# ishine/zerovox.cpp

Hardware: AMD Instinct MI355X
Metric: audio-seconds/wall-second (xRT) end-to-end phoneme->22.05 kHz wav (higher is better)
Workload: dtype f16*f16->f32 (MFMA) convs, f32 (MFMA) attention/linear, f32 activations

## Files before the change

### zerovox.cpp_amd/csrc/capi.cpp

```cpp
#include <algorithm>
#include <cmath>
#include <cstring>
#include <map>
#include <optional>
#include <string>
#include <thread>
#include <vector>

#include "common.h"
#include "model.h"
#include "knobs.h"

using zv::Model;

struct PendingBatch;
struct zv_model
{
    Model        *m;
    PendingBatch *pending;
};

static void free_pending(zv_model *m);
static void lane0_select(zv_model *m);
static void use_lane0(zv_model *m);
// ... 968 lines not shown
    if (env)
    {
        bt.d_env_gain = (const float *)(d_in + i_eg);
        bt.d_env = (const int32_t *)(d_in + i_env);
        bt.d_nframes = (const int32_t *)(io + o_nf);
    }
    int32_t *d_nf = (int32_t *)(io + o_nf), *d_ids = (int32_t *)(d_in + i_ids), *d_pun = (int32_t *)(d_in + i_pun);
    float *d_sty = (float *)(d_in + i_sty), *d_hid = (float *)(io + o_hid), *d_mel = (float *)(io + o_mel), *d_wav = (float *)(io + o_wav);
    int32_t *h_nf = (int32_t *)(pin + p_nf), *h_cum = dur ? (int32_t *)(pin + p_cum) : nullptr;
    char *h_wav = pin + p_wav;
    zv_level *h_lvl = vol ? (zv_level *)(pin + p_lvl) : nullptr;
    zv_frame_level *h_cfr = ctr_f ? (zv_frame_level *)(pin + p_cfr) : nullptr, *h_cph = ctr_p ? (zv_frame_level *)(pin + p_cph) : nullptr;
    zv_pitch_frame *h_pfr = pit_f ? (zv_pitch_frame *)(pin + p_pfr) : nullptr;
    zv_pitch_phoneme *h_pph = pit_p ? (zv_pitch_phoneme *)(pin + p_pph) : nullptr;
    float *h_bfr = bnd_f ? (float *)(pin + p_bfr) : nullptr, *h_bph = bnd_p ? (float *)(pin + p_bph) : nullptr;
    const size_t brs = zv::BANDS_ROW_STRIDE;
    auto contour_download = [&](uint32_t u0, uint32_t u1, hipStream_t st) {
        const size_t f0 = pb.woff[u0] / (hop * 4), f1 = u1 < r.count ? pb.woff[u1] / (hop * 4) : frame_rows;
        const size_t n0 = pb.noff[u0], n1 = pb.noff[u1];
        if (h_cfr && f1 > f0)
            ZV_HIP(hipMemcpyAsync(h_cfr + f0, bt.d_ctr_frames + f0, (f1 - f0) * sizeof(zv_frame_level), hipMemcpyDeviceToHost, st));
        if (h_cph && n1 > n0)
            ZV_HIP(hipMemcpyAsync(h_cph + n0, bt.d_ctr_phonemes + n0, (n1 - n0) * sizeof(zv_frame_level), hipMemcpyDeviceToHost, st));
        if (h_pfr && f1 > f0)
            ZV_HIP(hipMemcpyAsync(h_pfr + f0, bt.d_pit_frames + f0, (f1 - f0) * sizeof(zv_pitch_frame), hipMemcpyDeviceToHost, st));
        if (h_pph && n1 > n0)
            ZV_HIP(hipMemcpyAsync(h_pph + n0, bt.d_pit_phonemes + n0, (n1 - n0) * sizeof(zv_pitch_phoneme), hipMemcpyDeviceToHost, st));
        if (h_bfr && f1 > f0)
            ZV_HIP(hipMemcpyAsync(h_bfr + f0 * brs, bt.d_bnd_frames + f0 * brs, (f1 - f0) * brs * 4, hipMemcpyDeviceToHost, st));
        if (h_bph && n1 > n0)
            ZV_HIP(hipMemcpyAsync(h_bph + n0 * brs, bt.d_bnd_phonemes + n0 * brs, (n1 - n0) * brs * 4, hipMemcpyDeviceToHost, st));
    };
    const int G = zv::voc_tail_groups(bt.nseg, wav_bytes, M.profiling, M.dbg_layer.kind >= 0);
    try
    {
        hipStream_t cs = M.copy_stream();
        pb.gb.assign(G + 1, r.count);
        pb.gb[0] = 0;
        const uint64_t seq = M.next_batch_seq();
        ZV_HIP(hipEventRecord(M.batch_event(seq, 0), M.stream()));
        if (G <= 1)
        {
            M.chain_dev(bt, d_ids, d_pun, d_sty, d_hid, d_mel, d_wav, d_nf, h_in, d_in, b_in);
            ZV_HIP(hipEventRecord(M.batch_event(seq, 1), M.stream()));
            ZV_HIP(hipMemcpyAsync(h_nf, d_nf, (size_t)bt.nseg * 4, hipMemcpyDeviceToHost, M.stream()));
            if (dur) ZV_HIP(hipMemcpyAsync(h_cum, bt.d_cum, (size_t)ntot * 4, hipMemcpyDeviceToHost, M.stream()));
            ZV_HIP(hipMemcpyAsync(h_wav, d_wav, wav_bytes, hipMemcpyDeviceToHost, M.stream()));
            if (vol) ZV_HIP(hipMemcpyAsync(h_lvl, io + o_lvl, (size_t)bt.nseg * sizeof(zv_level), hipMemcpyDeviceToHost, M.stream()));
            contour_download(0, r.count, M.stream());
            ZV_HIP(hipEventRecord(M.tail_event(1), M.stream()));
        }
        else
        {
            M.chain_dev(bt, d_ids, d_pun, d_sty, d_hid, d_mel, d_wav, d_nf, h_in, d_in, b_in, 1);
            ZV_HIP(hipMemcpyAsync(h_nf, d_nf, (size_t)bt.nseg * 4, hipMemcpyDeviceToHost, M.stream()));
            if (dur) ZV_HIP(hipMemcpyAsync(h_cum, bt.d_cum, (size_t)ntot * 4, hipMemcpyDeviceToHost, M.stream()));
            for (int g = 1; g < G; g++)
            {
                uint32_t u = pb.gb[g - 1] + 1;
                while (u < r.count && pb.woff[u] < wav_bytes * g / G) u++;
                pb.gb[g] = std::min(u, r.count - (uint32_t)(G - g));
            }
            for (int g = 0; g < G; g++)
            {
                const uint32_t u0 = pb.gb[g], u1 = pb.gb[g + 1];
                M.vocode_tail(bt, d_mel, d_wav, (int)u0, (int)(u1 - u0));
                const size_t o0 = pb.woff[u0], o1 = u1 < r.count ? pb.woff[u1] : wav_bytes;
                ZV_HIP(hipEventRecord(M.tail_event(2 * g), M.stream()));
                ZV_HIP(hipStreamWaitEvent(cs, M.tail_event(2 * g), 0));
                ZV_HIP(hipMemcpyAsync(h_wav + o0, (const char *)d_wav + o0, o1 - o0, hipMemcpyDeviceToHost, cs));
                contour_download(u0, u1, cs);
                ZV_HIP(hipEventRecord(M.tail_event(2 * g + 1), cs));
            }
            ZV_HIP(hipEventRecord(M.batch_event(seq, 1), M.stream()));
            if (vol) ZV_HIP(hipMemcpyAsync(h_lvl, io + o_lvl, (size_t)bt.nseg * sizeof(zv_level), hipMemcpyDeviceToHost, M.stream()));
        }
    }
    catch (...)
    {
        hipStreamSynchronize(M.stream());
        if (M.copy_stream()) hipStreamSynchronize(M.copy_stream());
        throw;
    }
    pb.active = true;
    pb.n_utt = r.count;
    pb.G = G;
    pb.T.assign(r.T, r.T + r.count);
    pb.wav.assign(r.out, r.out + r.count);
    pb.n_frames = r.n_frames;
    pb.h_wav = h_wav;
    pb.h_nf = h_nf;
    pb.hop = hop;
    pb.h_cum = h_cum;
    pb.h_lvl = h_lvl;
    pb.levels = r.levels;
    pb.h_cfr = h_cfr;
    pb.h_cph = h_cph;
    if (ctr) pb.contour.assign(r.contour, r.contour + r.count);
    else pb.contour.clear();
    pb.h_pfr = h_pfr;
    pb.h_pph = h_pph;
    if (pit) pb.pitch.assign(r.pitch, r.pitch + r.count);
    else pb.pitch.clear();
    pb.h_bfr = h_bfr;
    pb.h_bph = h_bph;
    if (bnd) pb.bands.assign(r.bands, r.bands + r.count);
    else pb.bands.clear();
    pb.N.assign(r.n, r.n + r.count);
    if (dur) pb.dur.assign(r.durations, r.durations + r.count);
    else pb.dur.clear();
}

static void batch_finish(zv_model *m, int lane)
{
    Model &M = *m->m;
    PendingBatch &pb = pending_slot(m, lane);
    if (!pb.active) zv::fail(ZV_ERR_ARG, "lane %d has no batch in flight", lane);
    M.select_lane(lane);
    try
    {
        for (int g = 0; g < pb.G; g++)
        {
            ZV_HIP(hipEventSynchronize(M.tail_event(2 * g + 1)));
            scatter_out(pb.h_wav, pb.woff.data(), pb.wav.data(), pb.T.data(), pb.hop, pb.gb[g], pb.gb[g + 1]);
        }
        M.sync();
    }
    catch (...)
// ... 879 lines not shown
```

### zerovox.cpp_amd/csrc/knobs.h

```cpp
#pragma once

namespace zv
{

#define ZV_KNOB_LIST(X)                                                                                                               \
    X(ZV_NO_FUSE, 0)                                                                  \
    X(ZV_NO_TRIPLE, 0)                                                                          \
    X(ZV_FUSE256, 0)                                                \
    X(ZV_NO_MERGE, 0)                                                               \
    X(ZV_MERGE_ALWAYS, 0)                 \
    X(ZV_MERGE_SEQ, 1)          \
    X(ZV_MERGE_MAXC, 256)                                  \
    X(ZV_TAIL_GROUPS, 8)                                                        \
    X(ZV_ARENA_FILL, 0)                                         \
    X(ZV_DEC_PREPASS, -1)                                      \
    X(ZV_CONV_MT, 0)                                                              \
    X(ZV_CONV_NT, 0)                                                     \
    X(ZV_CONV_SINGLE, 1)                                    \
    X(ZV_CONV_GEMM, 1)                  \
    X(ZV_CONV_STREAM, 1)        \
    X(ZV_VOC_RUNS, 1)           \
    X(ZV_DEC_RUNS, 1)           \
    X(ZV_DEC_PACK, 1)           \
    X(ZV_UP_GEMM, 1)           \
    X(ZV_GEMM_ORDER, 2)         \
    X(ZV_PAIR_MT, 0)                                                                  \
    X(ZV_CONV_XCD, 1)           \
    X(ZV_CONV_WARM, 1)          \
    X(ZV_LINEAR_MERGED, 1)      \
    X(ZV_BLOCK64, 3)            \
    X(ZV_PAIR64_RING, 1)               \
    X(ZV_TRIPLE_V2, 1)                               \
    X(ZV_TRIPLE_DB, 1)                                                                     \
    X(ZV_TRIPLE_INTERLEAVE, 1)                                                               \
    X(ZV_ATT_SCALAR, 0)                                                                               \
    X(ZV_ATT_MFMA, 0)                                                          \
    X(ZV_LN_TAIL, 1)

#ifdef ZV_DIAG
#define ZV_KNOB_LIST_DIAG(X)                                                                                                          \
    X(ZV_DBG, 0)                                                                       \
    X(ZV_LDS_PAD, 0)            \
    X(ZV_STAMP_CP, 0)                               \
    X(ZV_STAMP_CONV, 0)                                    \
    X(ZV_STAMP_CIN, 0)
#else
#define ZV_KNOB_LIST_DIAG(X)
#endif

enum Knob : int
{
#define ZV_KNOB_ENUM(n, d) n,
    ZV_KNOB_LIST(ZV_KNOB_ENUM)
    ZV_KNOB_LIST_DIAG(ZV_KNOB_ENUM)
#undef ZV_KNOB_ENUM
    ZV_KNOB_COUNT
};

int         knob(Knob k);
bool        knob_set(const char *name, int value);
void        knob_reset();
bool        knob_get(const char *name, int *value);
unsigned    knob_epoch();
const char *knob_name(int k);
#ifdef ZV_DIAG
inline int diag_bits() { return knob(ZV_DBG); }
#else
// ... 5 lines not shown
```

### zerovox.cpp_amd/csrc/model.cpp

```cpp
#include "schedule.h"

#include <algorithm>

namespace zv
{

Model::~Model()
{
    hipSetDevice(device);
    for (Lane &l : lanes_) hipStreamSynchronize(l.stream);
    drop_graphs();
    prof_clear();
    for (void *p : allocs_) hipFree(p);
    for (hipEvent_t e : batch_events_)
        if (e) hipEventDestroy(e);
    for (Lane &l : lanes_)
    {
        if (l.copy_stream) hipStreamSynchronize(l.copy_stream);
        if (l.arena.base) hipFree(l.arena.base);
        if (l.io) hipFree(l.io);
        if (l.pinned) hipHostFree(l.pinned);
        for (hipEvent_t e : l.tail_events) hipEventDestroy(e);
        if (l.copy_stream) hipStreamDestroy(l.copy_stream);
        if (l.stream) hipStreamDestroy(l.stream);
// ... 233 lines not shown
    for (auto &g : graphs_)
        if (g.exec) hipGraphExecDestroy(g.exec);
    graphs_.clear();
}

template <typename F> void Model::run_captured(int kind, const Batch &b, const void *const (&key)[CapturedGraph::NKEY], F &&enqueue)
{
    for (auto &g : graphs_)
        if (g.kind == kind && g.epoch == knob_epoch() && b.same_schedule(g.b) && memcmp(g.p, key, sizeof(key)) == 0)
        {
            ZV_HIP(hipGraphLaunch(g.exec, stream()));
            lane().runs_tab = g.runs_tab;
            lane().runs_n = g.runs_n;
            return;
        }
    reserve_batch(b);
    hipGraph_t graph = nullptr;
    lane().runs_tab = nullptr;
    lane().runs_n = 0;
    ZV_HIP(hipStreamBeginCapture(stream(), hipStreamCaptureModeThreadLocal));
    try
    {
        enqueue();
    }
    catch (...)
    {
        hipStreamEndCapture(stream(), &graph);
        if (graph) hipGraphDestroy(graph);
        throw;
    }
    ZV_HIP(hipStreamEndCapture(stream(), &graph));
    CapturedGraph cg;
    cg.kind = kind;
    cg.epoch = knob_epoch();
    cg.b = b;
    memcpy(cg.p, key, sizeof(key));
    cg.runs_tab = lane().runs_tab;
    cg.runs_n = lane().runs_n;
    hipError_t e = hipGraphInstantiate(&cg.exec, graph, nullptr, nullptr, 0);
    hipGraphDestroy(graph);
    if (e != hipSuccess) fail(ZV_ERR_DEVICE, "hipGraphInstantiate failed: %s", hipGetErrorString(e));
    if (graphs_.size() >= 16)
    {
        ZV_HIP(hipStreamSynchronize(stream()));
        drop_graphs();
    }
    graphs_.push_back(cg);
    ZV_HIP(hipGraphLaunch(cg.exec, stream()));
}

void Model::chain_dev(const Batch &b, const int32_t *d_ids, const int32_t *d_puncts, const float *d_styles, float *d_hidden,
                      float *d_mel, float *d_wav, int32_t *d_nframes, const void *h2d_src, void *h2d_dst, size_t h2d_bytes, int voc_part)
{
    auto run = [&]() {
        if (h2d_bytes) ZV_HIP(hipMemcpyAsync(h2d_dst, h2d_src, h2d_bytes, hipMemcpyHostToDevice, stream()));
        encode_dev(b, d_ids, d_puncts, d_styles, d_hidden, d_nframes);
        decode_dev(b, d_hidden, d_styles, d_mel);
        if (voc_part == 1) vocode_group(b, d_mel, d_wav, 1);
        else vocode_dev(b, d_mel, d_wav);
    };
    if (!graph_mode || profiling) return run();
    const void *key[CapturedGraph::NKEY] = {d_ids, d_puncts, d_styles, d_hidden, d_mel, d_wav, d_nframes, h2d_src};
    run_captured(voc_part == 1 ? 2 : 1, b, key, run);
}

void Model::vocode_dev_graph(const Batch &b, const float *d_mel, float *d_wav)
{
    if (!graph_mode || profiling) return vocode_dev(b, d_mel, d_wav);
    const void *key[CapturedGraph::NKEY] = {d_mel, d_wav};
    run_captured(0, b, key, [&]() { vocode_dev(b, d_mel, d_wav); });
}

}
```

### zerovox.cpp_amd/csrc/model.h

```cpp
#pragma once

#include <cstdint>
#include <cstring>
#include <string>
#include <vector>

#include "common.h"
#include "gguf_reader.h"
#include "kernels.h"

namespace zv
{

struct ConvW
{
    void  *w = nullptr;
    void  *w8 = nullptr;
    float *bias = nullptr;
    int    K = 0, Cin = 0, Cout = 0, Cin_p = 0, Cout_p = 0, ck = 0;
};

struct DeviceArena
{
    char  *base = nullptr;
// ... 49 lines not shown
    const void         *d_bnd_table = nullptr;
    const uint32_t     *d_flt_par = nullptr;

    static Batch single(uint32_t N, uint32_t T, uint32_t num_phonemes)
    {
        Batch b;
        b.n_max = (int)N;
        b.n_real = (int)N;
        b.t_max = (int)T;
        b.n_rows = N;
        b.t_rows = T;
        b.tok1 = Seg{0, (int32_t)N, (int32_t)num_phonemes, 0};
        b.frm1 = Seg{0, (int32_t)T, 0, 0};
        return b;
    }
    Segs tokens() const { return Segs{d_tok, nseg, n_max, tok1}; }
    Segs tokens_merged() const { return d_tok ? Segs{d_tok + nseg, 1, (int)n_rows, tok1} : tokens(); }
    Segs frames_cap() const { return Segs{d_frm, nseg, t_max, frm1}; }
    Segs frames() const { return d_frm_live ? Segs{d_frm_live, nseg, t_max, frm1} : frames_cap(); }
    bool same_schedule(const Batch &o) const
    {
        return nseg == o.nseg && n_max == o.n_max && t_max == o.t_max && n_rows == o.n_rows && t_rows == o.t_rows && d_tok == o.d_tok &&
               d_frm == o.d_frm && (d_tok || memcmp(&tok1, &o.tok1, sizeof(Seg)) == 0) && (d_frm || memcmp(&frm1, &o.frm1, sizeof(Seg)) == 0) &&
               d_ctl == o.d_ctl && d_pctl == o.d_pctl && d_cum == o.d_cum && d_frm_live == o.d_frm_live && has_targets == o.has_targets &&
               d_dec_runs == o.d_dec_runs && d_vol == o.d_vol && d_levels == o.d_levels && d_nframes == o.d_nframes && d_env_gain == o.d_env_gain &&
               d_env == o.d_env && d_ctr_frames == o.d_ctr_frames && d_ctr_phonemes == o.d_ctr_phonemes &&
               d_pit_frames == o.d_pit_frames && d_pit_phonemes == o.d_pit_phonemes && d_pit_par == o.d_pit_par &&
               d_bnd_frames == o.d_bnd_frames && d_bnd_phonemes == o.d_bnd_phonemes && d_bnd_slab == o.d_bnd_slab && d_bnd_par == o.d_bnd_par &&
               d_bnd_table == o.d_bnd_table && d_flt_par == o.d_flt_par;
    }
};

struct CapturedGraph
{
    static constexpr int NKEY = 8;
    int            kind = 0;
    unsigned       epoch = 0;
    Batch          b;
    const void    *p[NKEY] = {};
    hipGraphExec_t exec = nullptr;
    const Seg     *runs_tab = nullptr;
    int            runs_n = 0;
};

class Model
{
  public:
    Model(const std::string &gguf_path, int device);
    ~Model();

    zv_hparams hp{};
    int        device = 0;
    int        n_cu = 256;
    hipStream_t stream() const { return lanes_[cur_lane_].stream; }

    void vocode_dev(const Batch &b, const float *d_mel, float *d_wav);
    void vocode_group(const Batch &b, const float *d_mel, float *d_wav, int part = 0, int seg0 = 0);
    void vocode_tail(const Batch &b, const float *d_mel, float *d_wav, int g0, int cnt);
    hipStream_t copy_stream();
    hipEvent_t  tail_event(int i);
    static constexpr int BATCH_RING = 64;
    uint64_t    next_batch_seq() { return batch_seq_++; }
    uint64_t    batch_seq() const { return batch_seq_; }
    hipEvent_t  batch_event(uint64_t seq, int which);
    void decode_dev(const Batch &b, const float *d_hidden, const float *d_styles, float *d_mel);
    struct EncoderTaps
    {
        float   *features = nullptr, *logdur = nullptr, *pitch = nullptr, *energy = nullptr;
        int32_t *pitch_bucket = nullptr, *energy_bucket = nullptr, *cum = nullptr;
    };
    EncoderTaps encode_dev(const Batch &b, const int32_t *d_ids, const int32_t *d_puncts, const float *d_styles,
                           float *d_hidden, int32_t *d_nframes);

    struct DebugLayer
    {
        int          kind = -1, index = 0;
        const float *x = nullptr;
        float       *out = nullptr;
        bool         done = false;
    } dbg_layer;

    uint32_t max_phonemes() const { return (uint32_t)enc_.posenc_rows; }
    void reserve(uint32_t max_phonemes, uint32_t max_frames);
    void reserve_batch(const Batch &b);
    int  voc_stage_rate(int stage) const;
    int  voc_stage_channels(int stage) const;
    uint32_t max_frames_per_utterance() const;
    int wemb_rows() const { return enc_.wemb_rows; }
    int pemb_rows() const { return enc_.pemb_rows; }
    uint32_t vocoder_halo_frames() const;
    bool voc_runs_off = false;
    bool voc_runs_on(const Batch &b) const;
    const Seg *voc_runs_last(int *n) { *n = lane().runs_n; return lane().runs_tab; }
    DecPlan dec_plan(const Batch &b) const
    {
        return zv::dec_plan(b.nseg, b.t_max, b.t_rows, b.d_frm_live != nullptr, dbg_layer.kind >= 0, b.d_dec_runs != nullptr);
    }
    int  dec_reach_frames() const;
    void sync();

    void select_lane(int i);
    int  selected_lane() const { return cur_lane_; }
    void sync_all_lanes();
    void poison_lane(int i, int byte, size_t filled[3]);

    const void *bands_table();

    void *io_scratch(size_t bytes);
    void *pinned_scratch(size_t bytes);

    bool graph_mode = false;
// ... 90 lines not shown
    };
    size_t level_slab_entries(const Batch &b) const;
    size_t env_knot_entries(const Batch &b) const;
    struct DecLayout
    {
        int    nblk, hs, ss;
        int    rows, nblk_all;
        float *h, *st_x, *st_t, *st_y, *st_a, *cat, *t1, *sc, *x0, *xa, *asr_t;
        double *part_t, *part_o; _Float16 *xa16, *t16, *xr16;
        float *mel_c;
    };
    struct EncLayout { int Vp; float *x, *y, *qkv, *o, *f, *va, *vb; _Float16 *hh; EncoderTaps t; };
    VocLayout voc_layout(DeviceArena &a, const Batch &b) const;
    DecLayout dec_layout(DeviceArena &a, const Batch &b) const;
    EncLayout enc_layout(DeviceArena &a, const Batch &b) const;
    static constexpr size_t ARENA_TAIL = (size_t)1 << 20;
    size_t arena_bytes_for(const Batch &b) const;
    void  arena_require(size_t bytes);
    DeviceArena &stage_arena(const Batch &b);

    void conv(const ConvJob *jobs, int n, const Segs &segs, int rate, const char *name, double bytes, double flops);
    void dbg_inject(void *dev, int ld, int cols, size_t rows);
    void dbg_extract(const void *dev, int ld, int cols, size_t rows);
    ConvJob job(const ConvW &w) const;
    void tick(hipEvent_t *e0);
    void tock(hipEvent_t e0, const char *name, double bytes, double flops);
    void group_begin();
    void group_end(const char *name);
    bool       in_group_ = false;
    hipEvent_t group_e0_ = nullptr;
    double     group_bytes_ = 0.0, group_flops_ = 0.0;
    int        group_n_ = 0;

    struct Lane
    {
        hipStream_t stream = nullptr;
        DeviceArena arena;
        void       *io = nullptr;
        size_t      io_cap = 0;
        void       *pinned = nullptr;
        size_t      pinned_cap = 0;
        hipStream_t copy_stream = nullptr;
        std::vector<hipEvent_t> tail_events;
        const Seg  *runs_tab = nullptr;
        int         runs_n = 0;
    };
    std::vector<Lane> lanes_;
    int  cur_lane_ = 0;
    Lane &lane() { return lanes_[cur_lane_]; }
    uint64_t   batch_seq_ = 0;
    hipEvent_t batch_events_[2 * BATCH_RING] = {};

    bool skip_launch_ = false;
    std::vector<CapturedGraph> graphs_;
    void drop_graphs();
    template <typename F> void run_captured(int kind, const Batch &b, const void *const (&key)[CapturedGraph::NKEY], F &&enqueue);
};

}
```

### zerovox.cpp_amd/csrc/voc_plan.h

```cpp
#pragma once

#include <stddef.h>

#include "conv_plan.h"
#include "knobs.h"

namespace zv
{

constexpr int VOC_MAX_STAGES = 8, VOC_MAX_DIL = 8, VOC_BRANCHES = 3;
struct VocPairGeom
{
    int  k1, k2;
    bool fused, ring, x16;
};
struct VocStageGeom
{
    int         scale;
    int         Cp;
    bool        up_gemm;
    int         up_Cin_p;
    VocPairGeom pair[VOC_BRANCHES][VOC_MAX_DIL];
};
struct VocGeom
// ... 53 lines not shown
    const long Lbatch = (long)c.t_max * rate * c.nseg;
    p.up_pass = !(i == 0 && c0_f16) && voc_up_gemm(s, L) && (size_t)s.up_Cin_p * 2 * L <= Lo * Cp * 4;

    p.all_fusable = true;
    for (int jb = 0; jb < VOC_BRANCHES; jb++)
        for (int d = 0; d < g.n_dil; d++) p.all_fusable = p.all_fusable && s.pair[jb][d].fused;
    p.enough_rows = Cp != 256 || knob(ZV_FUSE256) != 0 || (Lbatch / 54) * 3 >= (long)c.n_cu;
    p.fused = knob(ZV_NO_FUSE) == 0 && p.all_fusable && p.enough_rows;

    p.whole_block = p.fused && knob(ZV_NO_TRIPLE) == 0 && g.n_dil <= TRIPLE_MAX_DIL;
    for (int jb = 0; jb < VOC_BRANCHES && p.whole_block; jb++)
    {
        const int K = s.pair[jb][0].k1;
        p.whole_block = triple_supported(Cp, K, g.dil, g.n_dil);
        for (int d = 0; d < g.n_dil && p.whole_block; d++) p.whole_block = s.pair[jb][d].fused && s.pair[jb][d].k1 == K && s.pair[jb][d].k2 == K;
    }

    const int k64 = knob(ZV_BLOCK64), kmax64 = k64 < 0 ? -k64 : k64;
    if (p.fused && !p.whole_block && Cp == 64 && g.n_dil == 3 && kmax64 >= 3 && (k64 < 0 || Lbatch / 244 >= 4L * c.n_cu))
        for (int jb = 0; jb < VOC_BRANCHES; jb++)
        {
            const VocPairGeom *rp = s.pair[jb];
            const bool one_k = rp[1].k1 == rp[0].k1 && rp[0].k2 == rp[0].k1 && rp[1].k2 == rp[0].k1;
            p.block64[jb] = one_k && rp[0].k1 <= kmax64 && rp[0].ring && rp[1].ring && block64_supported(Cp, rp[0].k1, g.dil, 2);
        }

    const int  merge_tile = Cp >= 256 ? 54 : (Cp == 128 ? 118 : 246);
    const bool merge_pays = knob(ZV_MERGE_ALWAYS) != 0 || (Lbatch / merge_tile >= 4L * c.n_cu && Cp <= knob(ZV_MERGE_MAXC));
    const bool merge = p.fused && !p.whole_block && knob(ZV_NO_MERGE) == 0 && c.dbg_stage != i && merge_pays;
    p.merge = !merge ? VOC_MERGE_NONE : (Cp >= 256 && knob(ZV_MERGE_SEQ) != 0 ? VOC_MERGE_SEQ : VOC_MERGE_ONE);
    return p;
}

inline VocPlan voc_plan(const VocGeom &g, const VocCall &c)
{
    VocPlan p{};
    p.runs = voc_runs(c);
    p.c0_f16 = !c.dbg_active && g.n_up > 0 && voc_up_gemm(g.st[0], c.t_rows) && g.st[0].up_Cin_p == g.in_Cout_p;
    for (int i = 0; i < g.n_up; i++) p.st[i] = voc_plan_stage(g, i, c, p.c0_f16);
    return p;
}

constexpr size_t TAIL_GROUPS_MIN_BYTES = (size_t)16 << 20;
inline int voc_tail_groups(int sw, int nseg, size_t wav_bytes, bool profiling, bool dbg_active)
{
    if (sw <= 1 || nseg < 4 || wav_bytes < TAIL_GROUPS_MIN_BYTES || profiling || dbg_active) return 1;
    return sw < nseg / 2 ? sw : nseg / 2;
}
inline int voc_tail_groups(int nseg, size_t wav_bytes, bool profiling, bool dbg_active)
{
    return voc_tail_groups(knob(ZV_TAIL_GROUPS), nseg, wav_bytes, profiling, dbg_active);
}

}
```

### zerovox.cpp_amd/csrc/vocoder.cpp

```cpp
#include "schedule.h"

#include <algorithm>
#include <cmath>

namespace zv
{

uint32_t Model::vocoder_halo_frames() const
{
    double frames = (voc_.in_conv.K - 1) / 2;
    double rate = 1.0;
    for (int i = 0; i < voc_.n_up; i++)
    {
        frames += (double)voc_.ups[i].K / rate;
        rate *= voc_.scales[i];
        int reach = 0;
        for (int j = 0; j < voc_.n_rb; j++)
        {
            int r = 0;
            for (int d = 0; d < voc_.n_dil; d++)
            {
                const ResPair &rp = voc_.pairs[((size_t)i * voc_.n_rb + j) * voc_.n_dil + d];
                r += (rp.c1.K - 1) / 2 * voc_.dil[d] + (rp.c2.K - 1) / 2;
            }
// ... 18 lines not shown
{
    VocLayout v{};
    v.c0 = a.take_n<float>(bt.t_rows * voc_.in_conv.Cout_p);
    DeviceArena pool[2] = {DeviceArena::counter(), DeviceArena::counter()};
    for (int pass = 0; pass < 2; pass++)
    {
        size_t L = bt.t_rows, need[2] = {0, 0};
        for (int i = 0; i < voc_.n_up; i++)
        {
            DeviceArena &p = pool[i & 1];
            VocLayout::Stage &s = v.st[i];
            L *= voc_.scales[i];
            const size_t n = L * round_up(voc_.in_conv.Cout >> (i + 1), 16);
            p.used = 0;
            s.ub = p.take_n<float>(n);
            for (int j = 0; j < 3; j++) s.y[j] = p.take_n<float>(n);
            for (int j = 0; j < 3; j++) s.xt[j] = (_Float16 *)p.take_n<float>(n);
            need[i & 1] = std::max(need[i & 1], p.used);
        }
        for (int k = 0; k < 2 && pass == 0; k++) pool[k] = DeviceArena{(char *)a.take(need[k]), need[k], 0};
    }
    v.mel_c = a.take_n<float>(bt.t_rows * hp.audio_num_mels);
    v.eq = a.take_n<int32_t>(bt.t_rows);
    v.level_slab = a.take(level_slab_entries(bt) * 16);
    v.env_knots = a.take_n<uint32_t>(env_knot_entries(bt));
    v.contour_slab = a.take(bt.t_rows * 16);
    v.pitch_slab = a.take(bt.t_rows * sizeof(PitchSlabRow));
    v.filter_in = bt.d_flt_par ? a.take_n<float>(bt.t_rows * hp.audio_hop_size) : nullptr;
    v.runs = a.take_n<Seg>(bt.nseg);
    return v;
}

size_t Model::level_slab_entries(const Batch &bt) const
{
    return (bt.t_rows * hp.audio_hop_size + LEVEL_CHUNK_SAMPLES - 1) / LEVEL_CHUNK_SAMPLES + bt.t_rows / (size_t)std::max(bt.t_max, 1) + 1;
}

size_t Model::env_knot_entries(const Batch &bt) const { return bt.t_rows + bt.t_rows / (size_t)std::max(bt.t_max, 1) + 1; }

void Model::vocode_dev(const Batch &bt, const float *d_mel, float *d_wav)
{
    if (bt.t_rows == 0 || bt.t_max <= 0) fail(ZV_ERR_ARG, "T must be > 0");
    vocode_group(bt, d_mel, d_wav);
}

VocCall Model::voc_call(const Batch &bt) const
{
    return VocCall{bt.nseg, bt.t_max, bt.t_rows, n_cu, bt.d_frm_live != nullptr, voc_runs_off, dbg_layer.kind >= 0,
                   dbg_layer.kind == 0 ? dbg_layer.index / voc_.n_rb : -1};
}

bool Model::voc_runs_on(const Batch &bt) const { return voc_runs(voc_call(bt)); }

void Model::vocode_tail(const Batch &bt, const float *d_mel, float *d_wav, int g0, int cnt)
{
    if (!bt.d_frm || g0 < 0 || cnt < 1 || g0 + cnt > bt.nseg) fail(ZV_ERR_ARG, "internal: bad segment group");
    Batch sub = bt;
    sub.d_frm = bt.d_frm + g0;
    if (bt.d_frm_live) sub.d_frm_live = bt.d_frm_live + g0;
    if (bt.d_vol)
    {
        sub.d_vol = bt.d_vol + (size_t)g0 * LEVEL_VOL_STRIDE;
        sub.d_levels = bt.d_levels + g0;
    }
    if (bt.d_nframes) sub.d_nframes = bt.d_nframes + g0;
    if (bt.d_pit_par) sub.d_pit_par = bt.d_pit_par + (size_t)g0 * PITCH_PARAM_STRIDE;
    if (bt.d_bnd_par) sub.d_bnd_par = bt.d_bnd_par + (size_t)g0 * BANDS_PARAM_STRIDE;
    if (bt.d_flt_par) sub.d_flt_par = bt.d_flt_par + (size_t)g0 * FILTER_PARAM_STRIDE;
    if (bt.d_env) sub.d_env = bt.d_env + (size_t)g0 * ENV_CTL_STRIDE;
    sub.nseg = cnt;
    vocode_group(sub, d_mel, d_wav, 2, g0);
}

TripleJob Model::block_job(const ResPair *rp, int n_dil, bool ring, const float *y, float *out) const
{
    TripleJob t;
    memset(&t, 0, sizeof(t));
    t.y = y;
    t.out = out;
    t.n_dil = n_dil;
    t.Cp = rp[0].c1.Cout_p;
    t.K = rp[0].c1.K;
    t.slope = 0.1f;
    for (int d = 0; d < n_dil; d++)
    {
        t.w1[d] = ring ? rp[d].r1 : rp[d].p1;
        t.w2[d] = ring ? rp[d].r2 : rp[d].p2;
        if (!ring)
        {
            t.w1x[d] = rp[d].x1;
            t.w2x[d] = rp[d].x2;
        }
        t.b1[d] = rp[d].c1.bias;
        t.b2[d] = rp[d].c2.bias;
        t.dil[d] = voc_.dil[d];
    }
    return t;
}

Model::DilPairJobs Model::pair_jobs(const ResPair &rp, int dil, const float *yin, float *yout, _Float16 *xt, float *y) const
{
    DilPairJobs r;
    r.c1 = job(rp.c1);
    r.c1.x0 = yin;
    r.c1.pro = PRO_ACT;
    r.c1.slope = 0.1f;
    r.c1.dil = dil;
    r.c1.pad = (rp.c1.K - 1) / 2 * dil;
    r.c1.eact = 1;
    r.c1.oslope = 0.1f;
    r.c1.out_f16 = 1;
    r.c1.out = xt;
    r.c2 = job(rp.c2);
    r.c2.x0 = xt;
    r.c2.pro = PRO_RAW_F16;
    r.c2.res = yin;
    r.c2.ldres = rp.c1.Cout_p;
    r.c2.out = y;
    memset(&r.p, 0, sizeof(r.p));
    r.p.y = yin;
    r.p.out = yout;
    r.p.w1 = rp.x1;
    r.p.w2 = rp.x2;
    r.p.w1r = rp.r1;
    r.p.w2r = rp.r2;
    r.p.b1 = rp.c1.bias;
    r.p.b2 = rp.c2.bias;
    r.p.Cp = rp.c1.Cout_p;
    r.p.K = rp.c1.K;
    r.p.dil = dil;
    r.p.slope = 0.1f;
    return r;
}

void Model::vocode_group(const Batch &bt, const float *d_mel, float *d_wav, int part, int seg0)
{
    struct Unskip { bool &f; ~Unskip() { f = false; } } unskip{skip_launch_};
    skip_launch_ = part == 2;
    const VocLayout lay = voc_layout(stage_arena(bt), bt);
    const int M = hp.audio_num_mels;
    const VocPlan plan = voc_plan(voc_geom_, voc_call(bt));
    const bool runs = plan.runs;
    const Segs fr = runs ? Segs{lay.runs + seg0, bt.nseg, bt.t_max, bt.frm1} : bt.frames();
    if (part != 2)
    {
        lane().runs_tab = runs ? lay.runs : nullptr;
        lane().runs_n = runs ? bt.nseg : 0;
    }
    if (runs)
    {
        ZV_LAUNCH("voc_runs", 12.0 * bt.t_rows * M, 0.0,
                  launch_voc_runs(stream(), d_mel, M, lay.mel_c, lay.eq, lay.runs, bt.frames_cap(), (int)vocoder_halo_frames()));
        d_mel = lay.mel_c;
    }
    size_t L = bt.t_rows;
    double La = std::min((double)bt.t_rows, (double)bt.t_max * bt.nseg);
    if (runs && profiling)
    {
        std::vector<Seg> tab((size_t)bt.nseg);
        ZV_HIP(hipMemcpyAsync(tab.data(), lay.runs + seg0, tab.size() * sizeof(Seg), hipMemcpyDeviceToHost, stream()));
        ZV_HIP(hipStreamSynchronize(stream()));
        La = 0;
        for (const Seg &g : tab) La += g.rows;
    }
    int rate = 1;
    int C = voc_.in_conv.Cout;
    float *c0 = lay.c0;

    {
        ConvJob j = job(voc_.in_conv);
        j.x0 = d_mel;
        j.ldx = M;
        j.pro = PRO_MELNORM;
        j.pa = voc_.mean;
        j.pb = voc_.scale;
        j.out = c0;
        if (plan.c0_f16)
        {
            j.eact = 1;
            j.oslope = 0.1f;
            j.out_f16 = 1;
        }
        conv(&j, 1, fr, rate, "voc_input_conv", conv_bytes(La, M, C, j.K, false), conv_flops(La, M, C, j.K));
        if (dbg_layer.kind == ZV_LAYER_VOC_INPUT)
        {
            dbg_extract(c0, voc_.in_conv.Cout_p, C, L);
            return;
        }
    }

    const float third = (float)(1.0 / (float)voc_.n_rb);
    const float *prev_y[3] = {nullptr, nullptr, nullptr};
    const float *prev_merged = nullptr;
    for (int i = 0; i < voc_.n_up; i++)
    {
        const bool last_stage = i == voc_.n_up - 1;
        const VocStagePlan &sp = plan.st[i];
        skip_launch_ = part == 2;
        const int s = voc_.scales[i];
        const ConvW &up = voc_.ups[i];
        const int Cout = C >> 1, Cp = round_up(Cout, 16);
        const size_t Lo = L * s;
        float *ub = lay.st[i].ub;
        float *y[3] = {lay.st[i].y[0], lay.st[i].y[1], lay.st[i].y[2]};
        _Float16 *const *xt = lay.st[i].xt;

        {
            ConvJob j = job(up);
            j.slope = 0.1f;
            if (i == 0) { j.x0 = c0; j.pro = PRO_ACT; }
            else if (prev_merged) { j.x0 = prev_merged; j.pro = PRO_SCALE_ACT; j.pscale = third; }
            else { j.x0 = prev_y[0]; j.x1 = prev_y[1]; j.x2 = prev_y[2]; j.pro = PRO_SUM3_ACT; j.pscale = third; }
            const bool dbg_up = dbg_layer.kind == ZV_LAYER_VOC_UPSAMPLE && dbg_layer.index == i;
            if (dbg_up)
            {
                float *in = i == 0 ? c0 : const_cast<float *>(prev_merged ? prev_merged : prev_y[0]);
                dbg_inject(in, up.Cin_p, C, L);
                j.x0 = in;
                j.x1 = j.x2 = nullptr;
                if (i > 0) { j.pro = PRO_SCALE_ACT; j.pscale = 1.0f; }
            }
            j.out = ub;
            if (i == 0 && plan.c0_f16)
            {
                j.x0 = c0;
                j.pro = PRO_RAW_F16;
            }
            else if (sp.up_pass)
            {
                ZV_LAUNCH("voc_upsample", 0.0, 0.0, launch_act_f16(stream(), (const float *)j.x0, (const float *)j.x1, (const float *)j.x2,
                                                                   j.pro == PRO_ACT ? 1.0f : j.pscale, j.slope, xt[2], (size_t)L * up.Cin_p));
                j.x0 = xt[2];
                j.x1 = j.x2 = nullptr;
                j.pro = PRO_RAW_F16;
                j.pscale = 1.0f;
            }
            conv(&j, 1, fr, rate, "voc_upsample", 4.0 * La * C * (i == 0 ? 1 : 3) + 4.0 * La * s * Cout + 2.0 * C * Cout * 2 * s,
                 2.0 * La * C * Cout * 2 * s);
        }
        if (dbg_layer.kind == ZV_LAYER_VOC_UPSAMPLE && dbg_layer.index == i)
        {
            dbg_extract(ub, Cp, Cout, Lo);
            return;
        }
        skip_launch_ = (part == 1 && last_stage) || (part == 2 && !last_stage);
        L = Lo;
        La *= s;
        rate *= s;
        C = Cout;
        const bool dbg_here = dbg_layer.kind == 0 && dbg_layer.index / voc_.n_rb == i;
        if (dbg_here) dbg_inject(ub, Cp, Cout, L);
        const ResPair *const rps = &voc_.pairs[(size_t)i * voc_.n_rb * voc_.n_dil];
        const float *ycur[3] = {ub, ub, ub};
        const float *merged_sum = nullptr;
        auto block_cost = [&](const ResPair *rp, int n, double &bytes, double &flops) {
            for (int d = 0; d < n; d++)
            {
                bytes += conv_bytes(La, C, C, rp[d].c1.K, false) + conv_bytes(La, C, C, rp[d].c2.K, true);
                flops += conv_flops(La, C, C, rp[d].c1.K) + conv_flops(La, C, C, rp[d].c2.K);
            }
        };
        group_begin();
        if (sp.whole_block)
        {
            TripleJob tj[3];
            double bb = 0, ff = 0;
            for (int jb = 0; jb < 3; jb++)
            {
                tj[jb] = block_job(rps + jb * voc_.n_dil, voc_.n_dil, false, ub, y[jb]);
                block_cost(rps + jb * voc_.n_dil, voc_.n_dil, bb, ff);
                ycur[jb] = y[jb];
            }
            ZV_LAUNCH("voc_resblock_conv", bb, ff, launch_triple(stream(), tj, 3, n_cu, fr, rate));
        }
        {
            TripleJob tj[3];
            int nj = 0;
            double bb = 0, ff = 0;
            for (int jb = 0; jb < 3; jb++)
            {
                if (!sp.block64[jb]) continue;
                tj[nj++] = block_job(rps + jb * voc_.n_dil, 2, true, ub, (float *)xt[jb]);
                block_cost(rps + jb * voc_.n_dil, 2, bb, ff);
                ycur[jb] = (float *)xt[jb];
            }
            if (nj) ZV_LAUNCH("voc_resblock_conv", bb, ff, launch_block64(stream(), tj, nj, fr, rate));
        }
        for (int d = 0; d < voc_.n_dil && !sp.whole_block; d++)
        {
            ConvJob j1[3], j2[3];
            PairJob pj[3];
            double b1 = 0, f1 = 0, b2 = 0, f2 = 0;
            int npj = 0;
            for (int jb = 0; jb < 3; jb++)
            {
                if (sp.block64[jb] && d < 2) continue;
                const ResPair &rp = rps[jb * voc_.n_dil + d];
                float *yout = sp.fused ? ((d & 1) ? (float *)xt[jb] : y[jb]) : y[jb];
// ... 2 lines not shown
                j1[jb] = pq.c1;
                j2[jb] = pq.c2;
                pj[npj++] = pq.p;
                ycur[jb] = sp.fused ? yout : y[jb];
                b1 += conv_bytes(La, C, C, rp.c1.K, false);
                f1 += conv_flops(La, C, C, rp.c1.K);
                b2 += conv_bytes(La, C, C, rp.c2.K, true);
                f2 += conv_flops(La, C, C, rp.c2.K);
            }
            if (d == voc_.n_dil - 1 && sp.merge != VOC_MERGE_NONE)
            {
                bool ms_free = true;
                for (int q = 0; q < npj; q++) ms_free = ms_free && pj[0].out != pj[q].y;
                float *ms = ms_free ? pj[0].out : nullptr;
                if (!ms) fail(ZV_ERR_DEVICE, "internal: no free buffer for the merged MRF sum");
                if (sp.merge == VOC_MERGE_SEQ)
                {
                    for (int jb = 0; jb < 3; jb++)
                    {
                        PairJob q = pj[jb];
                        q.sum_out = ms;
                        q.sum_in = jb ? ms : nullptr;
                        ZV_LAUNCH("voc_resblock_conv", (b1 + b2) / 3, (f1 + f2) / 3, launch_pair(stream(), &q, 1, n_cu, fr, rate));
                    }
                }
                else
                    ZV_LAUNCH("voc_resblock_conv", b1 + b2, f1 + f2,
                              launch_pair(stream(), pj, npj, n_cu, fr, rate, ms));
                merged_sum = ms;
            }
            else if (sp.fused)
            {
                if (npj) ZV_LAUNCH("voc_resblock_conv", b1 + b2, f1 + f2, launch_pair(stream(), pj, npj, n_cu, fr, rate));
            }
            else
            {
                conv(j1, 3, fr, rate, "voc_resblock_conv", b1, f1);
                conv(j2, 3, fr, rate, "voc_resblock_conv", b2, f2);
            }
        }
        static const char *const rb_names[8] = {"voc_resblock_s0", "voc_resblock_s1", "voc_resblock_s2", "voc_resblock_s3",
                                                "voc_resblock_s4", "voc_resblock_s5", "voc_resblock_s6", "voc_resblock_s7"};
        group_end(rb_names[i < 8 ? i : 7]);
        if (dbg_here)
        {
            dbg_extract(ycur[dbg_layer.index % voc_.n_rb], Cp, Cout, L);
            return;
        }
        for (int jb = 0; jb < 3; jb++) y[jb] = const_cast<float *>(ycur[jb]);
        for (int jb = 0; jb < 3; jb++) prev_y[jb] = y[jb];
        prev_merged = merged_sum;
    }

    skip_launch_ = part == 1;
    const bool filtered = bt.d_flt_par && dbg_layer.kind < 0;
    float *const wav_out = d_wav;
    if (filtered) d_wav = lay.filter_in;
    {
        OutConvArgs a;
        a.x0 = prev_merged ? prev_merged : prev_y[0];
        a.x1 = prev_merged ? nullptr : prev_y[1];
        a.x2 = prev_merged ? nullptr : prev_y[2];
        a.ldx = round_up(C, 16);
        a.L = 0;
        a.C = C;
        a.K = voc_.out_K;
        a.pscale = third;
        a.slope = (float)1e-2;
        a.w = voc_.out_w;
        a.bias = voc_.out_b;
        a.out = d_wav;
        a.segs = fr;
        a.rate = rate;
        a.runs = runs;
        if (dbg_layer.kind == ZV_LAYER_VOC_OUTPUT)
        {
            float *in = const_cast<float *>(a.x0);
            dbg_inject(in, a.ldx, C, L);
            a.x1 = a.x2 = nullptr;
            a.pscale = 1.0f;
        }
        ZV_LAUNCH("voc_output_conv", 12.0 * La * C + 4.0 * La, 2.0 * La * C * a.K, launch_out_conv(stream(), a));
        if (runs) ZV_LAUNCH("voc_run_fill", 8.0 * (L - La), 0.0, launch_voc_run_fill(stream(), d_wav, fr, rate));
        if (dbg_layer.kind == ZV_LAYER_VOC_OUTPUT) dbg_extract(d_wav, 1, 1, L);
        if (bt.d_frm_live) ZV_LAUNCH("voc_zero_tail", 4.0 * La, 0.0, launch_zero_tail(stream(), d_wav, 1, bt.frames_cap(), fr, rate));
    }
    if (filtered)
    {
        if (!lay.filter_in) fail(ZV_ERR_DEVICE, "internal: a filter without its input region");
        const Segs cap = bt.frames_cap();
        const double cap_samples = std::min((double)bt.t_rows, (double)bt.t_max * bt.nseg) * rate;
        ZV_LAUNCH("voc_filter", 8.0 * cap_samples, 2.0 * 255.0 * cap_samples,
                  launch_filter(stream(), lay.filter_in, wav_out, bt.d_flt_par, cap, bt.frames(), rate));
        d_wav = wav_out;
    }

    if (bt.d_env && dbg_layer.kind < 0)
    {
        if (!bt.d_cum || !bt.d_nframes || !bt.d_env_gain) fail(ZV_ERR_DEVICE, "internal: an envelope without the scan, the frame counts or the gains");
        const Segs cap = bt.frames_cap();
        const Segs tk{bt.d_tok ? bt.d_tok + seg0 : nullptr, bt.nseg, bt.n_max, bt.tok1};
        if (bt.t_rows + (size_t)bt.nseg > env_knot_entries(bt)) fail(ZV_ERR_DEVICE, "internal: envelope knot table too small");
        const double cap_rows = std::min((double)bt.t_rows, (double)bt.t_max * bt.nseg);
        ZV_LAUNCH("voc_env_knots", 4.0 * (cap_rows + bt.nseg) + 8.0 * std::min((double)bt.n_rows, (double)bt.n_max * bt.nseg), 0.0,
                  launch_env_knots(stream(), bt.d_cum, bt.d_env_gain, bt.d_env, bt.d_nframes, lay.env_knots, tk, cap));
        ZV_LAUNCH("voc_env_apply", 8.0 * cap_rows * rate, 0.0,
                  launch_env_apply(stream(), d_wav, bt.d_nframes, lay.env_knots, bt.d_env, cap, rate));
// ... 67 lines not shown
```

Measured before the change: 35000.

## Add schedulable vocoder tail with optional copy-stream overlap and split last upsample

Replaces the fixed per-group vocoder tail loop with a step schedule. The schedule can place the output conv and a pre-run of the last upsample stage on the copy stream, so they overlap with resblock compute on the main stream. A stream-override scope and finer vocoder part enums allow the head to skip the last upsample. Both new behaviours sit behind knobs that default off, so by default the schedule reproduces the previous order, with a little added host work.

Measured after the change: 35030, median of 3. No clear change (+0.1%).

```diff
diff --git a/zerovox.cpp_amd/csrc/capi.cpp b/zerovox.cpp_amd/csrc/capi.cpp
--- a/zerovox.cpp_amd/csrc/capi.cpp
+++ b/zerovox.cpp_amd/csrc/capi.cpp
@@ -1044,7 +1044,11 @@
         }
         else
         {
-            M.chain_dev(bt, d_ids, d_pun, d_sty, d_hid, d_mel, d_wav, d_nf, h_in, d_in, b_in, 1);
+            const bool up_split = M.voc_tail_up(bt, G);
+            const zv::TailSchedule ts = zv::voc_tail_schedule(G, zv::knob(zv::ZV_TAIL_OVERLAP) != 0, up_split);
+            if (!ts.n) zv::fail(ZV_ERR_DEVICE, "internal: %d tail groups have no schedule", G);
+            M.tail_event(zv::voc_tail_events(G) - 1);
+            M.chain_dev(bt, d_ids, d_pun, d_sty, d_hid, d_mel, d_wav, d_nf, h_in, d_in, b_in, up_split ? Model::VOC_HEAD_NO_UP : Model::VOC_HEAD);
             ZV_HIP(hipMemcpyAsync(h_nf, d_nf, (size_t)bt.nseg * 4, hipMemcpyDeviceToHost, M.stream()));
             if (dur) ZV_HIP(hipMemcpyAsync(h_cum, bt.d_cum, (size_t)ntot * 4, hipMemcpyDeviceToHost, M.stream()));
             for (int g = 1; g < G; g++)
@@ -1053,19 +1057,42 @@
                 while (u < r.count && pb.woff[u] < wav_bytes * g / G) u++;
                 pb.gb[g] = std::min(u, r.count - (uint32_t)(G - g));
             }
-            for (int g = 0; g < G; g++)
+            for (int k = 0; k < ts.n; k++)
             {
-                const uint32_t u0 = pb.gb[g], u1 = pb.gb[g + 1];
-                M.vocode_tail(bt, d_mel, d_wav, (int)u0, (int)(u1 - u0));
-                const size_t o0 = pb.woff[u0], o1 = u1 < r.count ? pb.woff[u1] : wav_bytes;
-                ZV_HIP(hipEventRecord(M.tail_event(2 * g), M.stream()));
-                ZV_HIP(hipStreamWaitEvent(cs, M.tail_event(2 * g), 0));
-                ZV_HIP(hipMemcpyAsync(h_wav + o0, (const char *)d_wav + o0, o1 - o0, hipMemcpyDeviceToHost, cs));
-                contour_download(u0, u1, cs);
-                ZV_HIP(hipEventRecord(M.tail_event(2 * g + 1), cs));
+                const zv::TailStep &sp = ts.s[k];
+                hipStream_t st = sp.stream == zv::TAIL_COPY ? cs : M.stream();
+                hipEvent_t ev = sp.event == zv::TAIL_EV_DONE ? M.batch_event(seq, 1) : (sp.event >= 0 ? M.tail_event(sp.event) : nullptr);
+                const uint32_t u0 = sp.group >= 0 ? pb.gb[sp.group] : 0, u1 = sp.group >= 0 ? pb.gb[sp.group + 1] : 0;
+                switch (sp.op)
+                {
+                case zv::TAIL_UP:
+                case zv::TAIL_BLOCKS:
+                case zv::TAIL_OUTPUTS:
+                {
+                    Model::StreamScope on(M, st);
+                    const bool both = sp.op == zv::TAIL_BLOCKS && k + 1 < ts.n && ts.s[k + 1].op == zv::TAIL_OUTPUTS &&
+                                      ts.s[k + 1].group == sp.group && ts.s[k + 1].stream == sp.stream;
+                    M.vocode_tail(bt, d_mel, d_wav, (int)u0, (int)(u1 - u0),
+                                  both ? Model::VOC_TAIL
+                                       : (sp.op == zv::TAIL_UP ? Model::VOC_TAIL_UP : (sp.op == zv::TAIL_BLOCKS ? Model::VOC_TAIL_BLOCKS : Model::VOC_TAIL_OUTPUTS)));
+                    k += both;
+                    break;
+                }
+                case zv::TAIL_DOWNLOAD:
+                {
+                    const size_t o0 = pb.woff[u0], o1 = u1 < r.count ? pb.woff[u1] : wav_bytes;
+                    ZV_HIP(hipMemcpyAsync(h_wav + o0, (const char *)d_wav + o0, o1 - o0, hipMemcpyDeviceToHost, st));
+                    contour_download(u0, u1, st);
+                    break;
+                }
+                case zv::TAIL_WAIT: ZV_HIP(hipStreamWaitEvent(st, ev, 0)); break;
+                case zv::TAIL_RECORD: ZV_HIP(hipEventRecord(ev, st)); break;
+                case zv::TAIL_JOIN:
+                    if (vol) ZV_HIP(hipMemcpyAsync(h_lvl, io + o_lvl, (size_t)bt.nseg * sizeof(zv_level), hipMemcpyDeviceToHost, st));
+                    break;
+                default: zv::fail(ZV_ERR_DEVICE, "internal: unknown tail step %d", sp.op);
+                }
             }
-            ZV_HIP(hipEventRecord(M.batch_event(seq, 1), M.stream()));
-            if (vol) ZV_HIP(hipMemcpyAsync(h_lvl, io + o_lvl, (size_t)bt.nseg * sizeof(zv_level), hipMemcpyDeviceToHost, M.stream()));
         }
     }
     catch (...)
diff --git a/zerovox.cpp_amd/csrc/knobs.h b/zerovox.cpp_amd/csrc/knobs.h
--- a/zerovox.cpp_amd/csrc/knobs.h
+++ b/zerovox.cpp_amd/csrc/knobs.h
@@ -12,7 +12,9 @@
     X(ZV_MERGE_SEQ, 1)          \
     X(ZV_MERGE_MAXC, 256)                                  \
     X(ZV_TAIL_GROUPS, 8)                                                        \
-    X(ZV_ARENA_FILL, 0)                                         \
+    X(ZV_TAIL_OVERLAP, 0)       \
+    X(ZV_TAIL_UP, 0)            \
+    X(ZV_ARENA_FILL, 0)                                        \
     X(ZV_DEC_PREPASS, -1)                                      \
     X(ZV_CONV_MT, 0)                                                              \
     X(ZV_CONV_NT, 0)                                                     \
diff --git a/zerovox.cpp_amd/csrc/model.cpp b/zerovox.cpp_amd/csrc/model.cpp
--- a/zerovox.cpp_amd/csrc/model.cpp
+++ b/zerovox.cpp_amd/csrc/model.cpp
@@ -309,16 +309,18 @@
 void Model::chain_dev(const Batch &b, const int32_t *d_ids, const int32_t *d_puncts, const float *d_styles, float *d_hidden,
                       float *d_mel, float *d_wav, int32_t *d_nframes, const void *h2d_src, void *h2d_dst, size_t h2d_bytes, int voc_part)
 {
+    if (voc_part != VOC_ALL && voc_part != VOC_HEAD && voc_part != VOC_HEAD_NO_UP) fail(ZV_ERR_ARG, "internal: a chain runs a head piece of the vocoder");
+    const bool head = voc_part != VOC_ALL;
     auto run = [&]() {
         if (h2d_bytes) ZV_HIP(hipMemcpyAsync(h2d_dst, h2d_src, h2d_bytes, hipMemcpyHostToDevice, stream()));
         encode_dev(b, d_ids, d_puncts, d_styles, d_hidden, d_nframes);
         decode_dev(b, d_hidden, d_styles, d_mel);
-        if (voc_part == 1) vocode_group(b, d_mel, d_wav, 1);
+        if (head) vocode_group(b, d_mel, d_wav, voc_part);
         else vocode_dev(b, d_mel, d_wav);
     };
     if (!graph_mode || profiling) return run();
     const void *key[CapturedGraph::NKEY] = {d_ids, d_puncts, d_styles, d_hidden, d_mel, d_wav, d_nframes, h2d_src};
-    run_captured(voc_part == 1 ? 2 : 1, b, key, run);
+    run_captured(voc_part == VOC_HEAD_NO_UP ? 3 : (head ? 2 : 1), b, key, run);
 }
 
 void Model::vocode_dev_graph(const Batch &b, const float *d_mel, float *d_wav)
diff --git a/zerovox.cpp_amd/csrc/model.h b/zerovox.cpp_amd/csrc/model.h
--- a/zerovox.cpp_amd/csrc/model.h
+++ b/zerovox.cpp_amd/csrc/model.h
@@ -125,11 +125,34 @@
     zv_hparams hp{};
     int        device = 0;
     int        n_cu = 256;
-    hipStream_t stream() const { return lanes_[cur_lane_].stream; }
+    hipStream_t stream() const { return stream_override_ ? stream_override_ : lanes_[cur_lane_].stream; }
+    class StreamScope
+    {
+      public:
+        StreamScope(Model &m, hipStream_t s) : m_(m), old_(m.stream_override_) { m_.stream_override_ = s; }
+        ~StreamScope() { m_.stream_override_ = old_; }
+        StreamScope(const StreamScope &) = delete;
+        StreamScope &operator=(const StreamScope &) = delete;
+
+      private:
+        Model      &m_;
+        hipStream_t old_;
+    };
 
     void vocode_dev(const Batch &b, const float *d_mel, float *d_wav);
-    void vocode_group(const Batch &b, const float *d_mel, float *d_wav, int part = 0, int seg0 = 0);
-    void vocode_tail(const Batch &b, const float *d_mel, float *d_wav, int g0, int cnt);
+    enum VocPart
+    {
+        VOC_ALL = 0,
+        VOC_HEAD = 1,
+        VOC_TAIL = 2,
+        VOC_TAIL_UP = 3,
+        VOC_TAIL_BLOCKS = 4,
+        VOC_TAIL_OUTPUTS = 5,
+        VOC_HEAD_NO_UP = 6
+    };
+    void vocode_group(const Batch &b, const float *d_mel, float *d_wav, int part = VOC_ALL, int seg0 = 0, const VocPlan *head_plan = nullptr);
+    void vocode_tail(const Batch &b, const float *d_mel, float *d_wav, int g0, int cnt, int part = VOC_TAIL);
+    bool voc_tail_up(const Batch &b, int G) const;
     hipStream_t copy_stream();
     hipEvent_t  tail_event(int i);
     static constexpr int BATCH_RING = 64;
@@ -326,6 +349,7 @@
     hipEvent_t batch_events_[2 * BATCH_RING] = {};
 
     bool skip_launch_ = false;
+    hipStream_t stream_override_ = nullptr;
     std::vector<CapturedGraph> graphs_;
     void drop_graphs();
     template <typename F> void run_captured(int kind, const Batch &b, const void *const (&key)[CapturedGraph::NKEY], F &&enqueue);
diff --git a/zerovox.cpp_amd/csrc/voc_plan.h b/zerovox.cpp_amd/csrc/voc_plan.h
--- a/zerovox.cpp_amd/csrc/voc_plan.h
+++ b/zerovox.cpp_amd/csrc/voc_plan.h
@@ -129,4 +129,67 @@
     return voc_tail_groups(knob(ZV_TAIL_GROUPS), nseg, wav_bytes, profiling, dbg_active);
 }
 
+enum TailStream { TAIL_COMPUTE = 0, TAIL_COPY = 1 };
+enum TailOp { TAIL_UP, TAIL_BLOCKS, TAIL_OUTPUTS, TAIL_DOWNLOAD, TAIL_WAIT, TAIL_RECORD, TAIL_JOIN };
+constexpr int TAIL_EV_DONE = -1;
+constexpr int TAIL_MAX_GROUPS = 32;
+struct TailStep
+{
+    int stream, op;
+    int group;
+    int event;
+};
+struct TailSchedule
+{
+    int      n;
+    TailStep s[TAIL_MAX_GROUPS * 10 + 8];
+};
+inline int voc_tail_events(int G) { return 3 * G + 1; }
+
+inline TailSchedule voc_tail_schedule(int G, bool overlap, bool up_split)
+{
+    TailSchedule t{};
+    if (G < 1 || G > TAIL_MAX_GROUPS) return t;
+    auto put = [&t](int stream, int op, int group, int event) { t.s[t.n++] = TailStep{stream, op, group, event}; };
+    auto copy_up = [&](int g) {
+        put(TAIL_COPY, TAIL_UP, g, -1);
+        put(TAIL_COPY, TAIL_RECORD, -1, 2 * G + g);
+    };
+    if (overlap && up_split)
+    {
+        put(TAIL_COMPUTE, TAIL_RECORD, -1, 3 * G);
+        put(TAIL_COPY, TAIL_WAIT, -1, 3 * G);
+        for (int g = 0; g < 2 && g < G; g++) copy_up(g);
+    }
+    for (int g = 0; g < G; g++)
+    {
+        if (!overlap)
+        {
+            if (up_split) put(TAIL_COMPUTE, TAIL_UP, g, -1);
+            put(TAIL_COMPUTE, TAIL_BLOCKS, g, -1);
+            put(TAIL_COMPUTE, TAIL_OUTPUTS, g, -1);
+            put(TAIL_COMPUTE, TAIL_RECORD, -1, 2 * g);
+            put(TAIL_COPY, TAIL_WAIT, -1, 2 * g);
+            put(TAIL_COPY, TAIL_DOWNLOAD, g, -1);
+            put(TAIL_COPY, TAIL_RECORD, -1, 2 * g + 1);
+            continue;
+        }
+        if (up_split) put(TAIL_COMPUTE, TAIL_WAIT, -1, 2 * G + g);
+        put(TAIL_COMPUTE, TAIL_BLOCKS, g, -1);
+        put(TAIL_COMPUTE, TAIL_RECORD, -1, 2 * g);
+        put(TAIL_COPY, TAIL_WAIT, -1, 2 * g);
+        put(TAIL_COPY, TAIL_OUTPUTS, g, -1);
+        if (g == G - 1) put(TAIL_COPY, TAIL_RECORD, -1, TAIL_EV_DONE);
+        put(TAIL_COPY, TAIL_DOWNLOAD, g, -1);
+        put(TAIL_COPY, TAIL_RECORD, -1, 2 * g + 1);
+        if (up_split && g + 2 < G) copy_up(g + 2);
+    }
+    if (overlap) put(TAIL_COMPUTE, TAIL_WAIT, -1, 2 * (G - 1) + 1);
+    else put(TAIL_COMPUTE, TAIL_RECORD, -1, TAIL_EV_DONE);
+    put(TAIL_COMPUTE, TAIL_JOIN, -1, -1);
+    return t;
 }
+
+inline bool voc_tail_up(int sw, int G, bool last_up_pass) { return sw != 0 && G > 1 && !last_up_pass; }
+
+}
diff --git a/zerovox.cpp_amd/csrc/vocoder.cpp b/zerovox.cpp_amd/csrc/vocoder.cpp
--- a/zerovox.cpp_amd/csrc/vocoder.cpp
+++ b/zerovox.cpp_amd/csrc/vocoder.cpp
@@ -94,9 +94,16 @@
 
 bool Model::voc_runs_on(const Batch &bt) const { return voc_runs(voc_call(bt)); }
 
-void Model::vocode_tail(const Batch &bt, const float *d_mel, float *d_wav, int g0, int cnt)
+bool Model::voc_tail_up(const Batch &bt, int G) const
+{
+    if (voc_.n_up < 1) return false;
+    return zv::voc_tail_up(knob(ZV_TAIL_UP), G, voc_plan(voc_geom_, voc_call(bt)).st[voc_.n_up - 1].up_pass);
+}
+
+void Model::vocode_tail(const Batch &bt, const float *d_mel, float *d_wav, int g0, int cnt, int part)
 {
     if (!bt.d_frm || g0 < 0 || cnt < 1 || g0 + cnt > bt.nseg) fail(ZV_ERR_ARG, "internal: bad segment group");
+    if (part != VOC_TAIL && part != VOC_TAIL_UP && part != VOC_TAIL_BLOCKS && part != VOC_TAIL_OUTPUTS) fail(ZV_ERR_ARG, "internal: not a tail piece");
     Batch sub = bt;
     sub.d_frm = bt.d_frm + g0;
     if (bt.d_frm_live) sub.d_frm_live = bt.d_frm_live + g0;
@@ -111,7 +118,8 @@
     if (bt.d_flt_par) sub.d_flt_par = bt.d_flt_par + (size_t)g0 * FILTER_PARAM_STRIDE;
     if (bt.d_env) sub.d_env = bt.d_env + (size_t)g0 * ENV_CTL_STRIDE;
     sub.nseg = cnt;
-    vocode_group(sub, d_mel, d_wav, 2, g0);
+    const VocPlan head_plan = voc_plan(voc_geom_, voc_call(bt));
+    vocode_group(sub, d_mel, d_wav, part, g0, &head_plan);
 }
 
 TripleJob Model::block_job(const ResPair *rp, int n_dil, bool ring, const float *y, float *out) const
@@ -175,16 +183,21 @@
     return r;
 }
 
-void Model::vocode_group(const Batch &bt, const float *d_mel, float *d_wav, int part, int seg0)
+void Model::vocode_group(const Batch &bt, const float *d_mel, float *d_wav, int part, int seg0, const VocPlan *head_plan)
 {
     struct Unskip { bool &f; ~Unskip() { f = false; } } unskip{skip_launch_};
-    skip_launch_ = part == 2;
+    const bool head = part == VOC_ALL || part == VOC_HEAD || part == VOC_HEAD_NO_UP;
+    const bool do_last_up = part == VOC_ALL || part == VOC_HEAD || part == VOC_TAIL_UP;
+    const bool do_last_blocks = part == VOC_ALL || part == VOC_TAIL || part == VOC_TAIL_BLOCKS;
+    const bool do_outputs = part == VOC_ALL || part == VOC_TAIL || part == VOC_TAIL_OUTPUTS;
+    skip_launch_ = !head;
     const VocLayout lay = voc_layout(stage_arena(bt), bt);
     const int M = hp.audio_num_mels;
-    const VocPlan plan = voc_plan(voc_geom_, voc_call(bt));
+    VocPlan plan = voc_plan(voc_geom_, voc_call(bt));
+    for (int i = 0; head_plan && i + 1 < voc_.n_up; i++) plan.st[i] = head_plan->st[i];
     const bool runs = plan.runs;
     const Segs fr = runs ? Segs{lay.runs + seg0, bt.nseg, bt.t_max, bt.frm1} : bt.frames();
-    if (part != 2)
+    if (head)
     {
         lane().runs_tab = runs ? lay.runs : nullptr;
         lane().runs_n = runs ? bt.nseg : 0;
@@ -238,7 +251,7 @@
     {
         const bool last_stage = i == voc_.n_up - 1;
         const VocStagePlan &sp = plan.st[i];
-        skip_launch_ = part == 2;
+        skip_launch_ = !(last_stage ? do_last_up : head);
         const int s = voc_.scales[i];
         const ConvW &up = voc_.ups[i];
         const int Cout = C >> 1, Cp = round_up(Cout, 16);
@@ -285,7 +298,7 @@
             dbg_extract(ub, Cp, Cout, Lo);
             return;
         }
-        skip_launch_ = (part == 1 && last_stage) || (part == 2 && !last_stage);
+        skip_launch_ = !(last_stage ? do_last_blocks : head);
         L = Lo;
         La *= s;
         rate *= s;
@@ -394,7 +407,7 @@
         prev_merged = merged_sum;
     }
 
-    skip_launch_ = part == 1;
+    skip_launch_ = !do_outputs;
     const bool filtered = bt.d_flt_par && dbg_layer.kind < 0;
     float *const wav_out = d_wav;
     if (filtered) d_wav = lay.filter_in;
```
